# j-wilson/GPflowPILCO

Hardware: AMD Instinct MI355X
Metric: moment_matched_rollout_step_elements_per_sec (higher is better)
Workload: dtype f32; 1 GPU; C3 (BASELINE configs[2]): N=2000 d=8 D=8 H=40 fp32 drift moment-match step / closed rollout; recipe=baseline: BASELINE.md recipe: lengthscales log-U[0.3,3], GP-prior targets, fresh mu~U[0,1]^d / Sigm~; N=2000, d=8, D=8, H=40, B_per_gpu=256, B_total=256, B_this_rank=256, parallelism=dp1 over B (weak), recipe=baseline, steps_requested=418, diag_pairs=f64, offdiag_pairs=f32

## Files before the change

gpflowpilco_amd/csrc/mm_common.h:

```cpp
#pragma once
#include <stddef.h>
#include <stdint.h>
#include "../../include/gpflowpilco_mm.h"

static inline size_t mm_align_up(size_t x, size_t a) { return (x + a - 1) / a * a; }
static inline int mm_round_up_int(int x, int a) { return (x + a - 1) / a * a; }
static inline size_t mm_elem_size(int dtype) { return dtype == MM_F64 ? 8 : 4; }

#define MM_ISTAGE_NO_ROUTE (1 << 20)
#define MM_ISTAGE_ROUTE (1 << 21)
#define MM_ISTAGE_NO_M56 (1 << 22)
#define MM_ISTAGE_OLD_OFFDIAG (1 << 23)
#define MM_ISTAGE_OLD_SPOLY56 (1 << 24)

#define MM_PW_KERNELS 3

static inline int mm_num_pairs(int L, int flags) {
  return (flags & MM_FULL_OUTPUT_COV) ? L * (L + 1) / 2 : L;
}

static inline int mm_moment_deg(int d) { return d <= 8 ? 4 : 2; }
static inline long long mm_binom(int n, int k) {
  if (k < 0 || k > n) return 0;
  long long r = 1;
  for (int i = 1; i <= k; ++i) r = r * (n - k + i) / i;
  return r;
}
static inline int mm_mono_count(int n, int d) { return (int)mm_binom(d + n - 1, n); }
static inline int mm_mono_offset(int n, int d) { int o = 0; for (int m = 0; m < n; ++m) o += mm_mono_count(m, d); return o; }
static inline size_t mm_rank_table_entries(int d) {
  const int dk = d <= 8 ? 8 : 32, deg = mm_moment_deg(d);
  size_t n = 0, p = 1;
  for (int k = 1; k <= deg; ++k) { p *= dk; n += p; }
  return n;
}
static inline int mm_moment_cols(int d) { return mm_round_up_int(mm_mono_offset(mm_moment_deg(d) + 1, d), 16); }
static inline int mm_moment56_off5(int d) { return d <= 8 ? mm_round_up_int(mm_mono_count(4, d), 128) : 0; }
static inline int mm_moment56_off6(int d) { return d <= 8 ? mm_moment56_off5(d) + mm_round_up_int(mm_mono_count(5, d), 128) : 0; }
static inline int mm_moment56_cols(int d) { return d <= 8 ? mm_moment56_off6(d) + mm_round_up_int(mm_mono_count(6, d), 128) : 0; }
struct MMTab56 { int ins[6], last[6], n_i16, mult2, mult3, n_f32; size_t bytes; };
static inline MMTab56 mm_tab56(int d) {
  MMTab56 t;
  int o = 0;
  for (int m = 0; m < 6; ++m) { t.ins[m] = o; o += mm_mono_count(m, d) * 8; }
  for (int k = 0; k < 6; ++k) { t.last[k] = o; o += mm_mono_count(k, d); }
  t.n_i16 = mm_round_up_int(o, 8);
// ... 225 lines not shown
```

gpflowpilco_amd/csrc/mm_kernels.hip:

```cpp
#include <hip/hip_runtime.h>
#include <math.h>
#include "mm_common.h"
#include "mm_cost.h"
#include "mm_dev.h"
#include "mm_mono.h"

#include <mutex>
#include <unordered_map>
#include "mm_fork.h"

#define MM_ABI_VERSION 2

namespace {
struct MMForkKey {
  int dev; hipStream_t stream;
  bool operator==(const MMForkKey& o) const { return dev == o.dev && stream == o.stream; }
};
struct MMForkKeyHash {
  size_t operator()(const MMForkKey& k) const { return std::hash<const void*>()((const void*)k.stream) * 31u + (size_t)k.dev; }
};
std::mutex g_fork_mu;
std::unordered_map<MMForkKey, MMFork*, MMForkKeyHash> g_forks;

MMFork* mm_fork_lookup(hipStream_t stream, bool create) {
// ... 1108 lines not shown
    if (traj_Sigma) traj_Sigma[(size_t)b * d * d + idx] = (T)v;
  }
  if (lane < d) {
    const double v = (double)mu[(size_t)b * d + lane] + dt * (double)f1[(size_t)b * d + lane];
    mu_out[(size_t)b * d + lane] = (T)v;
    if (traj_mu) traj_mu[(size_t)b * d + lane] = (T)v;
  }
}

template <typename T>
__global__ __launch_bounds__(64) void k_expected_cost(int d, const T* __restrict__ mean, const T* __restrict__ cov,
                                                      const T* __restrict__ target, const T* __restrict__ precis,
                                                      T* __restrict__ cost) {
  extern __shared__ double smem[];
  mm_expected_cost_body<T>(d, mean, cov, target, precis, cost, (int)blockIdx.x, (int)threadIdx.x, smem);
}

extern "C" int mm_mfma_supported(int d);
int mm_mfma_num_slots(int Mp);
int mm_f64_num_slots(int Mp, int diag);
int mm_launch_qred_f64_both(const double* Zc, int Kz, const double* Cm, const double* beta, int M, int L, int Mp, int d, int P, int NS,
                            int Po, int B, int force_worst, const double* qhR, const double* qhC, const double* rowD,
                            const double* colD, const double* w64, const double* q64, const double* rowO, const double* colO,
                            double* partB, double* partC, hipStream_t stream, bool* launched);
int mm_launch_qred_f64(const double* Zc, int Kz, const double* Cm, const double* beta, int M, int L, int Mp, int d,
                       int P, int NS, int p0, int npairs, int B, int diag, int lowp, int force_worst,
                       const double* w, const double* q, const double* rowA, const double* colB,
                       double* partB, double* partC, hipStream_t stream);
int mm_launch_qred_mfma(const char* packed, const MMModelLayout& ml, char* ws, const MMWorkspaceLayout& wl,
                        int B, int L, int d, int flags, hipStream_t stream);
int mm_launch_route(const char* packed, const MMModelLayout& ml, char* ws, const MMWorkspaceLayout& wl, int B, int L, int M,
                    int d, int flags, int agg, double* out, int32_t* status, hipStream_t stream);
int mm_launch_moments(const char* packed, const MMModelLayout& ml, char* ws, const MMWorkspaceLayout& wl,
                      int B, int L, int d, const void* mu_f32, int flags, hipStream_t stream);

int mm_launch_pack56(char* packed, const MMModelLayout& lay, int L, int M, int d, const double* Z, hipStream_t s);

#define MM_CHECK_LAUNCH() do { hipError_t e_ = hipGetLastError(); if (e_ != hipSuccess) return (int)e_; } while (0)

static int mm_check_common(const void* packed, int L, int M, int d, int dtype, int B) {
  if (!packed) return MM_E_ARG;
  if (L <= 0 || M <= 0 || d <= 0 || B <= 0) return MM_E_ARG;
  if (d > MM_DMAX) return MM_E_DIM;
  if (dtype != MM_F32 && dtype != MM_F64) return MM_E_DTYPE;
  return 0;
}

static inline int mm_dk(int d) { return d <= 4 ? 4 : d <= 8 ? 8 : d <= 16 ? 16 : 32; }

extern "C" int mm_abi_version(void) { return MM_ABI_VERSION; }

extern "C" size_t mm_packed_model_bytes(int L, int M, int d, int dtype, int with_C) {
  if (L <= 0 || M <= 0 || d <= 0 || d > MM_DMAX) return 0;
  return mm_model_layout(L, M, d, dtype, with_C).total;
}

extern "C" size_t mm_workspace_bytes(int B, int L, int M, int d, int dtype, int flags) {
  if (B <= 0 || L <= 0 || M <= 0 || d <= 0 || d > MM_DMAX) return 0;
  return mm_workspace_layout(B, L, M, d, dtype, flags).total;
}

template <typename T>
static int mm_pack_model_t(char* packed, const MMModelLayout& lay, int L, int M, int d,
                           const double* Z, const double* ls, const double* var, const double* beta,
                           const double* C, const double* mean_c, hipStream_t s) {
  const int sorted = M > MM_SORT_MIN_M ? 1 : 0;
  if (sorted) {
// ... 78 lines not shown
      if (ns > nblk) ns = nblk;
      return ns < 1 ? 1 : ns;
    };
#define MM_PAIRVEC_ARGS                                                                                                     \
    (const double*)(packed + ml.Zt64), (const double*)(packed + ml.zbar), ls2, L, M, wl.Mp, d, wl.P, mu, pairmat,            \
    (const double*)(ws + wl.rho1), (double*)(ws + wl.rowD), (double*)(ws + wl.colD), (T*)(ws + wl.rowO), (T*)(ws + wl.colO), \
    (const double*)(ws + wl.w64), (double*)(ws + wl.whR), (double*)(ws + wl.whC), amax,                                      \
    (const double*)(ws + wl.q64), (double*)(ws + wl.qhR), (double*)(ws + wl.qhC), (flags & MM_MODEL_UNCERTAINTY) ? 1 : 0, nblk, \
    (const double*)(ws + wl.lq), (const double*)(packed + ml.beta64), (const double*)(packed + ml.zmax2),                       \
    ((sizeof(T) == 4 && d <= 8) ? (unsigned short*)(ws + wl.wsp) : (unsigned short*)nullptr),                                \
    (unsigned char*)(ws + wl.gflag), (float*)(ws + wl.gmax2), ((flags & (MM_FORCE_WORST_TIER | MM_ISTAGE_NO_M56)) ? 0 : 1)
    auto pairvec = [&](int p0, int npairs, hipStream_t st) {
      if (npairs <= 0) return;
      if constexpr (DK <= 8) {
        hipLaunchKernelGGL((k_pairvec_reg<T, DK>), dim3(nsplit_for(npairs), npairs, B), dim3(256), 0, st, MM_PAIRVEC_ARGS, p0);
      } else {
        hipLaunchKernelGGL((k_pairvec<T, DK>), dim3(nsplit_for(npairs), npairs, B), dim3(256), 0, st, MM_PAIRVEC_ARGS, p0);
      }
    };
    pairvec(0, L, s);
    MM_CHECK_LAUNCH();
    if (wl.Po > 0) {
      MMFork* fork = (joins && (long long)wl.P * B >= 512) ? mm_fork_get(s) : nullptr;
      hipStream_t s2 = s;
      if (fork) {
        hipError_t ef = hipEventRecord(fork->fork, s);
        if (ef == hipSuccess) ef = hipStreamWaitEvent(fork->s2, fork->fork, 0);
        if (ef != hipSuccess) return (int)ef;
        s2 = fork->s2;
      }
      pairvec(L, wl.Po, s2);
      int rcs = 0;
      { hipError_t e_ = hipGetLastError(); if (e_ != hipSuccess) rcs = (int)e_; }
      if (!rcs && sizeof(T) == 4) rcs = mm_launch_moments(packed, ml, ws, wl, B, L, d, (const void*)mu, flags, s2);
      if (fork) {
        hipError_t ej = hipEventRecord(fork->join, fork->s2);
        if (rcs) { if (ej == hipSuccess) (void)hipStreamWaitEvent(s, fork->join, 0); return rcs; }
        if (ej != hipSuccess) return (int)ej;
      }
      if (rcs) return rcs;
    }
#undef MM_PAIRVEC_ARGS
  }
  MM_CHECK_LAUNCH();
  return 0;
}

template <typename T, int DK>
static int mm_Q_reduce_t(const char* packed, const MMModelLayout& ml, bool has_C, char* ws, const MMWorkspaceLayout& wl,
                         int L, int M, int d, int B, int flags, double jitter, T* Sff, int32_t* status, hipStream_t s) {
  const int with_unc = (flags & MM_MODEL_UNCERTAINTY) ? 1 : 0;
  const int full = (flags & MM_FULL_OUTPUT_COV) ? 1 : 0;
  if (with_unc && !has_C) return MM_E_NO_C;
  const double* Cm = with_unc ? (const double*)(packed + ml.Cm) : nullptr;
  double* partB = (double*)(ws + wl.partB);
  double* partC = (double*)(ws + wl.partC);
  const int nrb = (wl.Mp + MM_GEN_ROWS - 1) / MM_GEN_ROWS, ncb = (wl.Mp + MM_GEN_COLS - 1) / MM_GEN_COLS;
  const bool generic = (flags & MM_FORCE_GENERIC) != 0;
  const bool use_mfma32 = sizeof(T) == 4 && !generic && mm_mfma_supported(d);
  const int ns_gen = nrb * ncb;
  const int nsB_diag = generic ? ns_gen : mm_f64_num_slots(wl.Mp, 1), nsC = nsB_diag;
  const int nsB_off = generic ? ns_gen : (sizeof(T) == 4 ? (use_mfma32 ? mm_mfma_num_slots(wl.Mp) : ns_gen)
                                                         : mm_f64_num_slots(wl.Mp, 0));
  int stages = flags & (MM_STAGE_DIAG | MM_STAGE_OFFDIAG | MM_STAGE_FINALIZE);
  if (!stages) stages = MM_STAGE_DIAG | MM_STAGE_OFFDIAG | MM_STAGE_FINALIZE;
  const bool routes = use_mfma32 && wl.Po > 0 && !(flags & (MM_FORCE_WORST_TIER | MM_NO_ROUTE));
  bool both = false;
// ... 224 lines not shown
```

gpflowpilco_amd/csrc/mm_moments.hip:

```cpp
#include <hip/hip_runtime.h>
#include <math.h>
#include "mm_common.h"
#include "mm_mono.h"

typedef double f64x4m __attribute__((ext_vector_type(4)));

#define MM_GEMM_RB 64
#define MM_GEMM_NB 128
#define MM_GEMM_KB 32
#define MM_GEMM_AS 34
#define MM_GEMM_BS 144

__device__ __forceinline__ void mm_decode_pair_m(int p, int L, int& a, int& a2) {
  int r = p - L, i = 0;
  while (r >= L - 1 - i) { r -= L - 1 - i; ++i; }
  a = i; a2 = i + 1 + r;
}

__global__ __launch_bounds__(256) __attribute__((amdgpu_waves_per_eu(2, 2))) void k_wmom_gemm(const double* __restrict__ whR, const double* __restrict__ whC,
                                                      const double* __restrict__ Zm, int KMp, int L, int Mp, int B, int Po,
                                                      int nrb, int ncb, int nwork, int col_deg3,
                                                      const unsigned int* __restrict__ amaxc, const double* __restrict__ zmax2,
                                                      const int* __restrict__ gperm, double* __restrict__ mom) {
  const int orig = blockIdx.x;
  const int xcd = orig & 7, slot = orig >> 3;
  const int qn = nwork >> 3, rn = nwork & 7;
  int wi = (xcd < rn ? xcd * (qn + 1) : rn * (qn + 1) + (xcd - rn) * qn) + slot;
  const int rb = wi % nrb; wi /= nrb;
  const int ks = wi % MM_MOM_SPLIT; wi /= MM_MOM_SPLIT;
  const int cb = wi % ncb; wi /= ncb;
  const int a = wi;
  const int R = (L - 1) * B;
  auto row_item = [&](int r, int& b, int& po, int& side, int& acol) {
    const int which = r / B;
    b = r - which * B;
    const int ap = which < a ? which : which + 1;
    const int lo = ap < a ? ap : a, hi = ap < a ? a : ap;
    po = lo * (L - 1) - lo * (lo - 1) / 2 + (hi - lo - 1);
    side = ap < a ? 1 : 0;
    acol = hi;
  };
  const double* tab = Zm + (size_t)a * Mp * KMp;
  const int tid = threadIdx.x, wv = tid >> 6, lane = tid & 63, l15 = lane & 15, kq = lane >> 4;
  const int* perm = nullptr;
  if (cb * MM_GEMM_NB >= col_deg3) {
    if (gperm != nullptr) {
      if (rb * MM_GEMM_RB >= gperm[(size_t)L * R + a]) return;
      perm = gperm + (size_t)a * R;
    } else {
      const int r = rb * MM_GEMM_RB + lane;
      bool c = false;
      if (amaxc != nullptr && r < R) {
        int b, po, side, acol;
        row_item(r, b, po, side, acol);
        c = mm_item_collapsed(amaxc[(size_t)b * Po + po]);
      }
      if (!__any(c)) return;
    }
  }
  const int kslice = Mp / MM_MOM_SPLIT;
  const int k_begin = ks * kslice, nkb = kslice / MM_GEMM_KB;

  __shared__ double As[MM_GEMM_RB * MM_GEMM_AS];
  __shared__ double Bs[MM_GEMM_KB * MM_GEMM_BS];

  const int ar = tid >> 2, ak = (tid & 3) * 8;
  int arow = rb * MM_GEMM_RB + ar;
  arow = arow < R ? arow : R - 1;
  int ab, apo, aside, aacol;
  row_item(perm ? perm[arow] : arow, ab, apo, aside, aacol);
  const double* aptr = (aside ? whC : whR) + ((size_t)ab * Po + apo) * Mp + k_begin + ak;

  const int bk = tid >> 3, bc = (tid & 7) * 16;
  const int col0 = cb * MM_GEMM_NB + bc;
  const bool bvalid = col0 < KMp;
  const double* bptr = tab + (size_t)(k_begin + bk) * KMp + (bvalid ? col0 : 0);
  double2 ra[4], rbv[8];
  auto load_regs = [&](int kb) {
    const double* ap = aptr + kb * MM_GEMM_KB;
#pragma unroll
    for (int i = 0; i < 4; ++i) ra[i] = *reinterpret_cast<const double2*>(ap + 2 * i);
    const double* bp = bptr + (size_t)kb * MM_GEMM_KB * KMp;
#pragma unroll
    for (int i = 0; i < 8; ++i) rbv[i] = *reinterpret_cast<const double2*>(bp + 2 * i);
  };
  f64x4m acc[4][2];
#pragma unroll
  for (int rt = 0; rt < 4; ++rt)
#pragma unroll
    for (int ct = 0; ct < 2; ++ct) acc[rt][ct] = (f64x4m){0.0, 0.0, 0.0, 0.0};

  load_regs(0);
  for (int kb = 0; kb < nkb; ++kb) {
    __syncthreads();
#pragma unroll
    for (int i = 0; i < 4; ++i) *reinterpret_cast<double2*>(&As[ar * MM_GEMM_AS + ak + 2 * i]) = ra[i];
#pragma unroll
    for (int i = 0; i < 8; ++i)
      *reinterpret_cast<double2*>(&Bs[bk * MM_GEMM_BS + bc + 2 * ((i + (tid & 7)) & 7)]) = bvalid ? rbv[i] : make_double2(0.0, 0.0);
    __syncthreads();
    load_regs(kb + 1 < nkb ? kb + 1 : kb);
#pragma unroll
    for (int s = 0; s < MM_GEMM_KB / 4; ++s) {
      double av[4], bv[2];
#pragma unroll
      for (int rt = 0; rt < 4; ++rt) av[rt] = As[(rt * 16 + l15) * MM_GEMM_AS + 4 * s + kq];
#pragma unroll
      for (int ct = 0; ct < 2; ++ct)
        bv[ct] = Bs[(4 * s + kq) * MM_GEMM_BS + wv * 32 + ct * 16 + 2 * (((l15 >> 1) + 2 * wv + ct) & 7) + (l15 & 1)];
#pragma unroll
      for (int rt = 0; rt < 4; ++rt)
#pragma unroll
        for (int ct = 0; ct < 2; ++ct)
          acc[rt][ct] = __builtin_amdgcn_mfma_f64_16x16x4f64(av[rt], bv[ct], acc[rt][ct], 0, 0, 0);
    }
  }
#pragma unroll
  for (int rt = 0; rt < 4; ++rt)
#pragma unroll
    for (int r = 0; r < 4; ++r) {
      const int row = rb * MM_GEMM_RB + rt * 16 + kq + 4 * r;
      if (row >= R) continue;
      int b, po, side, acol;
      row_item(perm ? perm[row] : row, b, po, side, acol);
      double* o = mom + ((((size_t)b * Po + po) * 2 + side) * MM_MOM_SPLIT + ks) * KMp;
#pragma unroll
      for (int ct = 0; ct < 2; ++ct) {
        const int col = cb * MM_GEMM_NB + wv * 32 + ct * 16 + l15;
        if (col < KMp) o[col] = acc[rt][ct][r];
      }
    }
}

__global__ __launch_bounds__(1024) void k_wmom_perm(const unsigned int* __restrict__ amaxc, const double* __restrict__ zmax2, int L, int B,
                                                    int Po, int* __restrict__ gperm) {
  const int a = blockIdx.x, tid = threadIdx.x, wv = tid >> 6, lane = tid & 63;
  const int R = (L - 1) * B;
  __shared__ int wsum[3][16];
  __shared__ int tot[3];
  int* out = gperm + (size_t)a * R;
  int cnt[3] = {0, 0, 0};
  auto cls_of = [&](int r) {
    const int which = r / B, b = r - which * B;
    const int ap = which < a ? which : which + 1;
    const int lo = ap < a ? ap : a, hi = ap < a ? a : ap;
    const int po = lo * (L - 1) - lo * (lo - 1) / 2 + (hi - lo - 1);
    const unsigned int ac = amaxc[(size_t)b * Po + po];
    const float x2 = mm_collapse_bound2(ac, zmax2[hi]);
    return !mm_item_collapsed(ac) ? 3 : (x2 > MM_C6_X5_2 ? 0 : (x2 > MM_C6_X4_2 ? 1 : 2));
  };
  for (int r = tid; r < R; r += 1024) { const int c = cls_of(r); if (c < 3) ++cnt[c]; }
#pragma unroll
  for (int c = 0; c < 3; ++c) {
#pragma unroll
    for (int off = 32; off > 0; off >>= 1) cnt[c] += __shfl_down(cnt[c], off, 64);
    if (lane == 0) wsum[c][wv] = cnt[c];
  }
  __syncthreads();
  if (tid < 3) { int t = 0; for (int w = 0; w < 16; ++w) t += wsum[tid][w]; tot[tid] = t; }
  __syncthreads();
  int ofs[3] = {0, tot[0], tot[0] + tot[1]};
  int ofs_n = 0;
// ... 19 lines not shown
      before[k] += wb; ctot[k] = ct;
      nfront_before += before[k]; nfront_tot += ct;
    }
    if (in) {
      if (c < 3) out[ofs[c] + before[c]] = r;
      else out[R - 1 - (ofs_n + (tid - nfront_before))] = r;
    }
    const int nin = R - r0 < 1024 ? R - r0 : 1024;
#pragma unroll
    for (int k = 0; k < 3; ++k) ofs[k] += ctot[k];
    ofs_n += nin - nfront_tot;
  }
  if (tid == 0) {
    gperm[(size_t)L * R + a] = tot[0] + tot[1] + tot[2];
    gperm[(size_t)L * R + L + a] = tot[0] + tot[1];
    gperm[(size_t)L * R + 2 * L + a] = tot[0];
  }
}

__device__ __forceinline__ double mm_block_sum256m(double v, double* red) {
#pragma unroll
  for (int off = 32; off > 0; off >>= 1) v += __shfl_down(v, off, 64);
  __syncthreads();
  if ((threadIdx.x & 63) == 0) red[threadIdx.x >> 6] = v;
  __syncthreads();
  return red[0] + red[1] + red[2] + red[3];
}

template <int DK, int LB>
__global__ __launch_bounds__(256) void k_spoly(const double* __restrict__ mom, int KMp, const double* __restrict__ pairmat,
                                               const double* __restrict__ zbar, const double* __restrict__ zmax2,
                                               const unsigned int* __restrict__ amax, const unsigned int* __restrict__ amaxc,
                                               const float* __restrict__ mu,
                                               int L, int d, int P, int deg, int allow_collapse,
                                               int off1, int off2, int off3, int off4, const short* __restrict__ rtab,
                                               double c0, double c1, double* __restrict__ s12) {
  extern __shared__ double sm[];
  const int po = blockIdx.x, b = blockIdx.y, tid = threadIdx.x;
  const int Po = P - L, p = L + po;
  int a, a2;
  mm_decode_pair_m(p, L, a, a2);
  const int dn = 1 << (LB * deg);
#define MM_PADI(i_) ((i_) + ((i_) >> 5))
  double* T = sm;
  double* U = T + MM_PADI(dn);
  double* nh = U + MM_PADI(dn >> LB);
  double* qh = nh + KMp;
  double* Gs = qh + KMp;
  double* dmu = Gs + DK * DK;
  __shared__ double red[4];
  {
    const double* nm = mom + (((size_t)b * Po + po) * 2 + 0) * MM_MOM_SPLIT * KMp;
    const double* qm = mom + (((size_t)b * Po + po) * 2 + 1) * MM_MOM_SPLIT * KMp;
    for (int k = tid; k < KMp; k += 256) {
      double sn = 0.0, sq = 0.0;
#pragma unroll
      for (int t = 0; t < MM_MOM_SPLIT; ++t) { sn += nm[t * KMp + k]; sq += qm[t * KMp + k]; }
      nh[k] = sn; qh[k] = sq;
    }
    const double* pm = pairmat + ((size_t)b * P + p) * (d * d + 1);
    for (int idx = tid; idx < DK * DK; idx += 256) {
      const int i = idx >> LB, j = idx & (DK - 1);
      Gs[idx] = (i < d && j < d) ? pm[i * d + j] : 0.0;
    }
    const bool rcen = mm_rows_recentred(amax[(size_t)b * Po + po]);
    if (tid < DK) dmu[tid] = (tid < d && !rcen) ? (double)mu[(size_t)b * d + tid] - zbar[a * d + tid] : 0.0;
  }
  __syncthreads();
  const bool coll = allow_collapse && deg >= 3 && mm_item_collapsed(amaxc[(size_t)b * Po + po]);
  const int nmax = coll ? deg : 2;
  double Gr[DK == 8 ? 64 : 1];
  if constexpr (DK == 8) {
#pragma unroll
    for (int i = 0; i < 64; ++i) Gr[i] = Gs[i];
  }
  double total = 0.0;
  for (int n = nmax; n >= 1; --n) {
    const double an = n == 1 ? 1.0 : n == 2 ? 0.5 : n == 3 ? c0 : c1;
    const int dsz = 1 << (LB * n);
    const int offn = n == 1 ? off1 : n == 2 ? off2 : n == 3 ? off3 : off4;
    const short* rtn = rtab + (((1 << (LB * n)) - DK) / (DK - 1));
    for (int idx = tid; idx < dsz; idx += 256) {
      const int r = rtn[idx];
      T[MM_PADI(idx)] = r >= 0 ? qh[offn + r] : 0.0;
    }
    __syncthreads();
    for (int t = 0; t < n; ++t) {
      const int sh = LB * t, nfib = dsz >> LB;
      for (int f = tid; f < nfib; f += 256) {
        const int lo = f & ((1 << sh) - 1), hi = f >> sh;
        const int base = (hi << (sh + LB)) + lo;
        double v[DK];
#pragma unroll
        for (int l = 0; l < DK; ++l) v[l] = T[MM_PADI(base + (l << sh))];
        if constexpr (DK == 8) {
#pragma unroll
          for (int k = 0; k < 8; ++k) {
            double s = 0.0;
#pragma unroll
            for (int l = 0; l < 8; ++l) s = fma(Gr[k * 8 + l], v[l], s);
            T[MM_PADI(base + (k << sh))] = s;
          }
        } else {
// ... 18 lines not shown
      const short* rtk = rtab + (k ? (((1 << (LB * k)) - DK) / (DK - 1)) : 0);
      for (int idx = tid; idx < ksz; idx += 256) {
        const int r = k ? rtk[idx] : 0;
        if (r >= 0) part = fma(cur[MM_PADI(idx)], nh[offk + r], part);
      }
      total = fma(an * sign_binom, part, total);
      if (k == 0) break;
      const int nsz = ksz >> LB;
      for (int idx = tid; idx < nsz; idx += 256) {
        double s = 0.0;
#pragma unroll
        for (int l = 0; l < DK; ++l) s = fma(cur[MM_PADI(l * nsz + idx)], dmu[l], s);
        oth[MM_PADI(idx)] = s;
      }
      __syncthreads();
      double* tsw = cur; cur = oth; oth = tsw;
      ksz = nsz;
      sign_binom = -sign_binom * (double)k / (double)(n - k + 1);
    }
    __syncthreads();
  }
  const double tot = mm_block_sum256m(total, red);
  if (tid == 0) s12[(size_t)b * Po + po] = tot + nh[0] * qh[0];
#undef MM_PADI
}

int mm_launch_wmom_full(const char* packed, const MMModelLayout& ml, char* ws, const MMWorkspaceLayout& wl,
                        int B, int L, int d, hipStream_t stream) {
  const int nrb = ((L - 1) * B + MM_GEMM_RB - 1) / MM_GEMM_RB, ncb = (ml.KMp + MM_GEMM_NB - 1) / MM_GEMM_NB;
  const long long nwork_ll = (long long)L * ncb * MM_MOM_SPLIT * nrb;
  if (nwork_ll <= 0 || nwork_ll > 0x7fffffffLL) return MM_E_DIM;
  hipLaunchKernelGGL(k_wmom_gemm, dim3((int)nwork_ll), dim3(256), 0, stream, (const double*)(ws + wl.whR),
                     (const double*)(ws + wl.whC), (const double*)(packed + ml.Zm), ml.KMp, L, wl.Mp, B, wl.Po, nrb, ncb,
                     (int)nwork_ll, 0x7fffffff , (const unsigned int*)nullptr, (const double*)(packed + ml.zmax2),
                     (const int*)nullptr, (double*)(ws + wl.mom));
  hipError_t e = hipGetLastError();
  return e == hipSuccess ? 0 : (int)e;
}

int mm_launch_moments56(const char* packed, const MMModelLayout& ml, char* ws, const MMWorkspaceLayout& wl,
                        int B, int L, int d, int allow, int old_spoly56, hipStream_t stream);

int mm_launch_moments(const char* packed, const MMModelLayout& ml, char* ws, const MMWorkspaceLayout& wl,
                      int B, int L, int d, const void* mu_f32, int flags, hipStream_t stream) {
  const double* Zm = (const double*)(packed + ml.Zm);
  double* mom = (double*)(ws + wl.mom);
  const int deg = mm_moment_deg(d) >= 4 ? 3 : mm_moment_deg(d);
  const int ncol_fwd = mm_mono_offset(deg + 1, d);
  const int nrb = ((L - 1) * B + MM_GEMM_RB - 1) / MM_GEMM_RB, ncb = (ncol_fwd + MM_GEMM_NB - 1) / MM_GEMM_NB;
  const long long nwork_ll = (long long)L * ncb * MM_MOM_SPLIT * nrb;
  if (nwork_ll <= 0 || nwork_ll > 0x7fffffffLL) return MM_E_DIM;
  const int nwork = (int)nwork_ll;
  const int allow = (flags & (MM_FORCE_WORST_TIER | MM_ISTAGE_NO_M56)) ? 0 : 1;
  const int col_deg3 = mm_mono_offset(3, d);
  const bool some = allow && mm_moment_deg(d) >= 4;
  if (some) {
    hipLaunchKernelGGL(k_wmom_perm, dim3(L), dim3(1024), 0, stream, (const unsigned int*)(ws + wl.amaxc),
                       (const double*)(packed + ml.zmax2), L, B, wl.Po, (int*)(ws + wl.gperm));
    hipError_t ep = hipGetLastError();
    if (ep != hipSuccess) return (int)ep;
  }
  hipLaunchKernelGGL(k_wmom_gemm, dim3(nwork), dim3(256), 0, stream, (const double*)(ws + wl.whR),
                     (const double*)(ws + wl.whC), Zm, ml.KMp, L, wl.Mp, B, wl.Po, nrb, ncb, nwork, col_deg3,
                     some ? (const unsigned int*)(ws + wl.amaxc) : (const unsigned int*)nullptr,
                     (const double*)(packed + ml.zmax2), some ? (const int*)(ws + wl.gperm) : (const int*)nullptr, mom);
  hipError_t e = hipGetLastError();
  if (e != hipSuccess) return (int)e;
  const int off1 = mm_mono_offset(1, d), off2 = mm_mono_offset(2, d), off3 = mm_mono_offset(3, d), off4 = mm_mono_offset(4, d);
#define MM_SPOLY(DK_, LB_)                                                                                                       \
  do {                                                                                                                          \
    const int dn_ = 1 << (LB_ * deg);                                                                                           \
    const int up_ = dn_ >> LB_;                                                                                                 \
    const size_t shm_ = (size_t)(dn_ + (dn_ >> 5) + up_ + (up_ >> 5) + 2 * ml.KMp + DK_ * DK_ + DK_ + 8) * sizeof(double);      \
    hipLaunchKernelGGL((k_spoly<DK_, LB_>), dim3(wl.Po, B), dim3(256), shm_, stream, (const double*)mom, ml.KMp,                \
                       (const double*)(ws + wl.pairmat), (const double*)(packed + ml.zbar), (const double*)(packed + ml.zmax2), \
                       (const unsigned int*)(ws + wl.amax), (const unsigned int*)(ws + wl.amaxc), (const float*)mu_f32, L, d, wl.P, deg, allow, off1, off2, off3, off4, \
                       (const short*)(packed + ml.rtab),                                                                        \
                       (double)MM_C6_C0, (double)MM_C6_C1, (double*)(ws + wl.s12));                                             \
  } while (0)
  if (d <= 8) MM_SPOLY(8, 3); else MM_SPOLY(32, 5);
#undef MM_SPOLY
  e = hipGetLastError();
  if (e != hipSuccess) return (int)e;
  if (flags & MM_ISTAGE_NO_M56) {
    if (mm_moment56_cols(d) <= 0 || wl.Po <= 0) return 0;
    const hipError_t em = hipMemsetAsync(ws + wl.s56, 0xFF, (size_t)B * wl.Po * sizeof(double), stream);
    if (em != hipSuccess) return (int)em;
    const hipError_t es = hipMemsetAsync(ws + wl.estS, 0, (size_t)B * wl.Po * sizeof(float), stream);
    return es == hipSuccess ? 0 : (int)es;
  }
  return mm_launch_moments56(packed, ml, ws, wl, B, L, d, some ? 1 : 0, (flags & MM_ISTAGE_OLD_SPOLY56) ? 1 : 0, stream);
}

__global__ void k_offdiag_stats(const unsigned int* __restrict__ amax, const double* __restrict__ zmax2,
                                const unsigned char* __restrict__ gflag, int ng, int L, int Po, int n,
                                int32_t* __restrict__ out) {
  const int idx = blockIdx.x * blockDim.x + threadIdx.x;
  bool c = false, in = false, part = false;
  int groups = 0;
  if (idx < n) {
    int a, a2;
    mm_decode_pair_m(L + idx % Po, L, a, a2);
    const float b2 = mm_collapse_bound2(amax[idx], zmax2[a2]);
    c = b2 <= MM_COLLAPSE_BOUND2;
    in = b2 <= MM_INSIDE_BOUND2;
    part = !c && mm_item_collapsed(amax[n + idx]);
    for (int g = 0; g < ng; ++g) groups += gflag[(size_t)idx * ng + g] ? 1 : 0;
  }
  const unsigned long long m = __ballot(c), mi = __ballot(in), mp = __ballot(part);
  if ((threadIdx.x & 63) == 0 && m) atomicAdd(out, (int)__popcll(m));
  if ((threadIdx.x & 63) == 0 && mi) atomicAdd(out + 2, (int)__popcll(mi));
  if ((threadIdx.x & 63) == 0 && mp) atomicAdd(out + 4, (int)__popcll(mp));
#pragma unroll
  for (int off = 32; off > 0; off >>= 1) groups += __shfl_down(groups, off, 64);
  if ((threadIdx.x & 63) == 0 && groups) atomicAdd(out + 5, groups);
  if (idx == 0) out[1] = n;
}

extern "C" int mm_offdiag_stats(const void* packed, size_t packed_bytes, int L, int M, int d, int dtype, int B, int flags,
                                const void* workspace, size_t workspace_bytes, int32_t* out, void* stream) {
  if (!packed || !workspace || !out || L <= 0 || M <= 0 || d <= 0 || d > MM_DMAX || B <= 0) return MM_E_ARG;
  const MMModelLayout ml = mm_model_layout(L, M, d, dtype, 1);
  const MMWorkspaceLayout wl = mm_workspace_layout(B, L, M, d, dtype, flags);
  if (packed_bytes < ml.Cm || workspace_bytes < wl.total) return MM_E_WORKSPACE;
// ... 16 lines not shown
```

gpflowpilco_amd/csrc/mm_moments6.hip:

```cpp
#include <hip/hip_runtime.h>
#include <math.h>
#include "mm_common.h"
#include "mm_mono.h"
#include "mm_f32_tile.h"
#include <atomic>
#include <type_traits>

__device__ __forceinline__ void mm6_decode_pair_o(int lp, int L, int& a, int& a2) {
  int r = lp, i = 0;
  while (r >= L - 1 - i) { r -= L - 1 - i; ++i; }
  a = i; a2 = i + 1 + r;
}

__global__ __launch_bounds__(256) void k_pack_zm56(char* packed, MMModelLayout lay, int L, int M, int d, int N56p,
                                                   const double* __restrict__ Z) {
  const int c = blockIdx.x, a = blockIdx.y, tid = threadIdx.x;
  const int n4 = mm_binom_i(d + 3, 4), n5 = mm_binom_i(d + 4, 5), n6 = mm_binom_i(d + 5, 6);
  const int off5 = ((n4 + 127) / 128) * 128;
  const int off6 = off5 + ((n5 + 127) / 128) * 128;
  const double* zbar = (const double*)(packed + lay.zbar) + (size_t)a * d;
  unsigned short* oh = (unsigned short*)(packed + lay.Zm56) + (((size_t)a * 2 + 0) * N56p + c) * lay.Mp;
  unsigned short* om = (unsigned short*)(packed + lay.Zm56) + (((size_t)a * 2 + 1) * N56p + c) * lay.Mp;
  int n = 0, k[6] = {0, 0, 0, 0, 0, 0};
  if (c < n4) { n = 4; mm_mono_unrank(c, 4, k); }
// ... 43 lines not shown
  for (int n = 2; n <= 3; ++n) {
    const int ns = mm_binom_i(d + n - 1, n);
    for (int I = tid; I < ns; I += 256) {
      int k[6] = {0, 0, 0, 0, 0, 0};
      mm_mono_unrank(I, n, k);
      double mult = 1.0;
      int run = 0;
      for (int u = 0; u < n; ++u) {
        mult *= (double)(u + 1);
        run = (u > 0 && k[u] == k[u - 1]) ? run + 1 : 1;
        mult /= (double)run;
      }
      f32[(n == 2 ? t.mult2 : t.mult3) + I] = (float)mult;
    }
  }
}

int mm_launch_pack56(char* packed, const MMModelLayout& lay, int L, int M, int d, const double* Z, hipStream_t s) {
  const int N56p = mm_moment56_cols(d);
  if (N56p <= 0) return 0;
  hipLaunchKernelGGL(k_pack_zm56, dim3(N56p, L), dim3(256), 0, s, packed, lay, L, M, d, N56p, Z);
  hipError_t e = hipGetLastError();
  if (e != hipSuccess) return (int)e;
  hipLaunchKernelGGL(k_pack_tab56, dim3(1), dim3(256), 0, s, packed, lay, d, mm_tab56(d));
  e = hipGetLastError();
  return e == hipSuccess ? 0 : (int)e;
}

#define MM6_TB 128
#define MM6_KB 32
#define MM6_STAGE_BYTES 32768

__global__ __launch_bounds__(256, 2) void k_wmom56_gemm(const unsigned short* __restrict__ wsp, const unsigned short* __restrict__ Zm56,
                                                        int N56p, int L, int Mp, int B, int Po, int nrb, int ncb, int nwork, int cb5, int cb6,
                                                        const int* __restrict__ gperm, float* __restrict__ mom56) {
  const int orig = blockIdx.x;
  const int xcd = orig & 7, slot = orig >> 3;
  const int qn = nwork >> 3, rn = nwork & 7;
  int wi = (xcd < rn ? xcd * (qn + 1) : rn * (qn + 1) + (xcd - rn) * qn) + slot;
  const int rb = wi % nrb; wi /= nrb;
  const int cb = wi % ncb; wi /= ncb;
  const int a = wi;
  const int R = (L - 1) * B;
  const int ncoll = gperm[(size_t)L * R + (cb < cb5 ? 0 : (cb < cb6 ? 1 : 2)) * L + a];
  if (rb * MM6_TB >= ncoll) return;
  const int* perm = gperm + (size_t)a * R;
  extern __shared__ __align__(1024) char lds[];
  int* orow = reinterpret_cast<int*>(lds + 2 * MM6_STAGE_BYTES);
  const int tid = threadIdx.x, wv = tid >> 6, lane = tid & 63, l31 = lane & 31, h = lane >> 5;
  auto row_item = [&](int r) {
    const int which = r / B, b = r - which * B;
    const int ap = which < a ? which : which + 1;
    const int lo = ap < a ? ap : a, hi = ap < a ? a : ap;
    const int po = lo * (L - 1) - lo * (lo - 1) / 2 + (hi - lo - 1);
    return ((b * Po + po) << 1) | (ap < a ? 1 : 0);
  };
  if (tid < MM6_TB) {
    const int r = rb * MM6_TB + tid;
    orow[tid] = r < ncoll ? row_item(perm[r]) : -1;
  }
  const bool isB = wv >= 2;
  const int part = wv & 1;
  unsigned int src_off[8];
#pragma unroll
  for (int i = 0; i < 8; ++i) {
    const int row = i * 16 + (lane >> 2);
    const int lc = (lane & 3) ^ ((row >> 2) & 3);
    if (isB) {
      src_off[i] = (unsigned int)((((size_t)a * 2 + part) * N56p + (size_t)cb * MM6_TB + row) * Mp) + lc * 8;
    } else {
      int r = rb * MM6_TB + row;
      r = r < ncoll ? r : ncoll - 1;
      src_off[i] = (unsigned int)(((size_t)row_item(perm[r]) * 2 + part) * Mp) + lc * 8;
    }
  }
  const unsigned short* src = isB ? Zm56 : wsp;
  auto stage = [&](int kb, int buf) {
    char* dst = lds + buf * MM6_STAGE_BYTES + (isB ? 16384 : 0) + part * 8192;
#pragma unroll
    for (int i = 0; i < 8; ++i)
      __builtin_amdgcn_global_load_lds((const __attribute__((address_space(1))) void*)(src + src_off[i] + kb * MM6_KB),
                                       (__attribute__((address_space(3))) void*)(dst + i * 1024), 16, 0, 0);
  };
  const int wr = wv >> 1, wc = wv & 1;
  f32x16 acc[2][2];
#pragma unroll
  for (int rt = 0; rt < 2; ++rt)
#pragma unroll
    for (int ct = 0; ct < 2; ++ct)
#pragma unroll
      for (int e = 0; e < 16; ++e) acc[rt][ct][e] = 0.0f;
  int fragA[2], fragB[2];
#pragma unroll
  for (int t = 0; t < 2; ++t) {
    fragA[t] = (wr * 64 + t * 32 + l31) * 64;
    fragB[t] = 16384 + (wc * 64 + t * 32 + l31) * 64;
  }
  const int swz = (l31 >> 2) & 3;
  const int nkb = Mp / MM6_KB;
  stage(0, 0);
  for (int kb = 0; kb < nkb; ++kb) {
    __syncthreads();
    if (kb + 1 < nkb) stage(kb + 1, (kb + 1) & 1);
    const char* base = lds + (kb & 1) * MM6_STAGE_BYTES;
#pragma unroll
    for (int ks = 0; ks < 2; ++ks) {
      const int ch = ((ks * 2 + h) ^ swz) * 16;
      bf16x8 Ah[2], Am[2], Th[2], Tm[2];
#pragma unroll
      for (int t = 0; t < 2; ++t) {
        Ah[t] = *reinterpret_cast<const bf16x8*>(base + fragA[t] + ch);
        Am[t] = *reinterpret_cast<const bf16x8*>(base + 8192 + fragA[t] + ch);
        Th[t] = *reinterpret_cast<const bf16x8*>(base + fragB[t] + ch);
        Tm[t] = *reinterpret_cast<const bf16x8*>(base + 8192 + fragB[t] + ch);
      }
#pragma unroll
      for (int rt = 0; rt < 2; ++rt)
#pragma unroll
        for (int ct = 0; ct < 2; ++ct) {
          acc[rt][ct] = __builtin_amdgcn_mfma_f32_32x32x16_bf16(Am[rt], Th[ct], acc[rt][ct], 0, 0, 0);
          acc[rt][ct] = __builtin_amdgcn_mfma_f32_32x32x16_bf16(Ah[rt], Tm[ct], acc[rt][ct], 0, 0, 0);
          acc[rt][ct] = __builtin_amdgcn_mfma_f32_32x32x16_bf16(Ah[rt], Th[ct], acc[rt][ct], 0, 0, 0);
        }
    }
  }
#pragma unroll
  for (int rt = 0; rt < 2; ++rt)
#pragma unroll
    for (int e = 0; e < 16; ++e) {
      const int item = orow[wr * 64 + rt * 32 + 8 * (e >> 2) + 4 * h + (e & 3)];
      if (item < 0) continue;
      float* o = mom56 + (size_t)item * N56p + (size_t)cb * MM6_TB + wc * 64 + l31;
// ... 488 lines not shown
        G[4 * q] = g4.x; G[4 * q + 1] = g4.y; G[4 * q + 2] = g4.z; G[4 * q + 3] = g4.w;
      }
    };
    float acc4 = 0.0f, dummy = 0.0f;
    const float* Q4 = nq + sy[4];
    const float* N4 = nq;
    load_G(1);
    mm6_do<D8, 0, false, 0, NC0, NW, 4, 0>(Q4, Bf4, sy, tabi, tb, d, G, nullptr, 0, dummy, wave, lane);
    __syncthreads();
    mm6_do<D8, 1, false, 1, 1, NW, 3, 37>(Bf4, X4, sy, tabi, tb, d, G, mult2, xs4, dummy, wave, lane);
    __syncthreads();
    load_G(0);
    mm6_do<D8, 0, true, 0, NC0, NW, 4, 0>(N4, Bf4, sy, tabi, tb, d, G, nullptr, 0, dummy, wave, lane);
    __syncthreads();
    mm6_do<D8, 1, true, 2, 1, NW, 3, 37>(Bf4, X4, sy, tabi, tb, d, G, nullptr, xs4, acc4, wave, lane);
    double tot = (double)MM_C6_C1 * (double)acc4;
#pragma unroll
    for (int off = 32; off > 0; off >>= 1) {
      tot += __shfl_down(tot, off, 64); s2r += __shfl_down(s2r, off, 64); s2c += __shfl_down(s2c, off, 64);
    }
    if (lane == 0) { redd[wave * 3 + 0] = tot; redd[wave * 3 + 1] = s2r; redd[wave * 3 + 2] = s2c; }
    __syncthreads();
    if (tid == 0) {
      double t = 0.0, r2 = 0.0, c2 = 0.0;
      for (int w = 0; w < NW; ++w) { t += redd[w * 3]; r2 += redd[w * 3 + 1]; c2 += redd[w * 3 + 2]; }
      s56[item] = t;
      estS[item] = mm6_estS(bound2, false, false, r2, c2);
    }
    __syncthreads();
  }
}

int mm_launch_moments56(const char* packed, const MMModelLayout& ml, char* ws, const MMWorkspaceLayout& wl,
                        int B, int L, int d, int allow, int old_spoly56, hipStream_t stream) {
  const int N56p = mm_moment56_cols(d);
  if (N56p <= 0 || wl.Po <= 0) return 0;
  if (allow) {
    const int nrb = ((L - 1) * B + MM6_TB - 1) / MM6_TB, ncb = N56p / MM6_TB;
    const long long nwork_ll = (long long)L * ncb * nrb;
    if (nwork_ll <= 0 || nwork_ll > 0x7fffffffLL) return MM_E_DIM;
    if ((size_t)B * wl.Po * 4 * wl.Mp >= 0xffffffffull || (size_t)L * 2 * N56p * wl.Mp >= 0xffffffffull) return MM_E_DIM;
    const size_t shm = 2 * MM6_STAGE_BYTES + MM6_TB * sizeof(int);
    static std::atomic<unsigned long long> attr_done{0ull};
    int dev = 0;
    if (hipGetDevice(&dev) != hipSuccess) dev = 64;
    const unsigned long long bit = (dev >= 0 && dev < 64) ? (1ull << dev) : 0ull;
    if (!bit || !(attr_done.load() & bit)) {
      const hipError_t ea = hipFuncSetAttribute((const void*)k_wmom56_gemm, hipFuncAttributeMaxDynamicSharedMemorySize, (int)shm);
      if (ea != hipSuccess) return (int)ea;
      attr_done.fetch_or(bit);
    }
    hipLaunchKernelGGL(k_wmom56_gemm, dim3((int)nwork_ll), dim3(256), shm, stream, (const unsigned short*)(ws + wl.wsp),
                       (const unsigned short*)(packed + ml.Zm56), N56p, L, wl.Mp, B, wl.Po, nrb, ncb, (int)nwork_ll,
                       mm_moment56_off5(d) / MM6_TB, mm_moment56_off6(d) / MM6_TB,
                       (const int*)(ws + wl.gperm), (float*)(ws + wl.mom56));
    hipError_t e = hipGetLastError();
    if (e != hipSuccess) return (int)e;
  }
  const int nitem = B * wl.Po;
  int* ilist = (int*)(ws + wl.ilist);
  {
    const hipError_t em = hipMemsetAsync(ilist, 0, 16, stream);
    if (em != hipSuccess) return (int)em;
  }
  hipLaunchKernelGGL(k_item_classes, dim3((nitem + 255) / 256), dim3(256), 0, stream, (const unsigned int*)(ws + wl.amaxc),
                     (const double*)(packed + ml.zmax2), L, wl.Po, nitem, allow, ilist, (double*)(ws + wl.s56), (float*)(ws + wl.estS));
  {
    const hipError_t ec = hipGetLastError();
    if (ec != hipSuccess) return (int)ec;
  }
  if (!allow) return 0;
  int sy[7];
  for (int k = 0; k < 7; ++k) sy[k] = mm_mono_count(k, d);
  size_t nfl = (size_t)2 * (sy[4] + sy[5] + sy[6]) + (size_t)sy[3] * (sy[3] + 1) + (size_t)sy[2] * sy[4] + (size_t)sy[1] * sy[5] + 6 * MM6_WAVES + 128 + 16
               + (size_t)sy[1] * sy[3] + (size_t)sy[2] * (sy[2] + 1);
  nfl = (nfl + 1) & ~(size_t)1;
  const size_t shm = nfl * sizeof(float);
  static std::atomic<unsigned long long> attr2_done{0ull};
  static std::atomic<int> ncu_cached[64];
  int dev = 0;
  if (hipGetDevice(&dev) != hipSuccess) dev = 64;
  const unsigned long long bit2 = (dev >= 0 && dev < 64) ? (1ull << dev) : 0ull;
  int ncu = bit2 ? ncu_cached[dev].load() : 0;
  if (!bit2 || !(attr2_done.load() & bit2)) {
    hipError_t ea = hipFuncSetAttribute((const void*)k_spoly56<false>, hipFuncAttributeMaxDynamicSharedMemorySize, 160 * 1024);
    if (ea == hipSuccess) ea = hipFuncSetAttribute((const void*)k_spoly56<true>, hipFuncAttributeMaxDynamicSharedMemorySize, 160 * 1024);
// ... 27 lines not shown
```

Before: 42100 rollout step-elements/s (B*H per rollout second).

## Trim moment GEMMs to live K rows and live monomial columns

The f64 moment GEMM and the bf16 56-moment GEMM now stop their K loop at the real inducing-point count M instead of the padded Mp. The f64 GEMM also limits its columns to the live monomial count, using a light single-row-tile MFMA path when few column tiles remain. The spoly reduction reads only up to the needed monomial offset. This removes wasted MFMA work and memory traffic on padding, at the cost of more branching and per-wave divergence in tile counts. An escape flag keeps the old extents available.

```diff
diff --git a/gpflowpilco_amd/csrc/mm_common.h b/gpflowpilco_amd/csrc/mm_common.h
--- a/gpflowpilco_amd/csrc/mm_common.h
+++ b/gpflowpilco_amd/csrc/mm_common.h
@@ -12,6 +12,7 @@
 #define MM_ISTAGE_NO_M56 (1 << 22)
 #define MM_ISTAGE_OLD_OFFDIAG (1 << 23)
 #define MM_ISTAGE_OLD_SPOLY56 (1 << 24)
+#define MM_ISTAGE_OLD_EXTENT (1 << 25)
 
 #define MM_PW_KERNELS 3
 
diff --git a/gpflowpilco_amd/csrc/mm_kernels.hip b/gpflowpilco_amd/csrc/mm_kernels.hip
--- a/gpflowpilco_amd/csrc/mm_kernels.hip
+++ b/gpflowpilco_amd/csrc/mm_kernels.hip
@@ -1164,7 +1164,7 @@
 int mm_launch_route(const char* packed, const MMModelLayout& ml, char* ws, const MMWorkspaceLayout& wl, int B, int L, int M,
                     int d, int flags, int agg, double* out, int32_t* status, hipStream_t stream);
 int mm_launch_moments(const char* packed, const MMModelLayout& ml, char* ws, const MMWorkspaceLayout& wl,
-                      int B, int L, int d, const void* mu_f32, int flags, hipStream_t stream);
+                      int B, int L, int M, int d, const void* mu_f32, int flags, hipStream_t stream);
 
 int mm_launch_pack56(char* packed, const MMModelLayout& lay, int L, int M, int d, const double* Z, hipStream_t s);
 
@@ -1309,7 +1309,7 @@
       pairvec(L, wl.Po, s2);
       int rcs = 0;
       { hipError_t e_ = hipGetLastError(); if (e_ != hipSuccess) rcs = (int)e_; }
-      if (!rcs && sizeof(T) == 4) rcs = mm_launch_moments(packed, ml, ws, wl, B, L, d, (const void*)mu, flags, s2);
+      if (!rcs && sizeof(T) == 4) rcs = mm_launch_moments(packed, ml, ws, wl, B, L, M, d, (const void*)mu, flags, s2);
       if (fork) {
         hipError_t ej = hipEventRecord(fork->join, fork->s2);
         if (rcs) { if (ej == hipSuccess) (void)hipStreamWaitEvent(s, fork->join, 0); return rcs; }
diff --git a/gpflowpilco_amd/csrc/mm_moments.hip b/gpflowpilco_amd/csrc/mm_moments.hip
--- a/gpflowpilco_amd/csrc/mm_moments.hip
+++ b/gpflowpilco_amd/csrc/mm_moments.hip
@@ -2,6 +2,7 @@
 #include <math.h>
 #include "mm_common.h"
 #include "mm_mono.h"
+#include <type_traits>
 
 typedef double f64x4m __attribute__((ext_vector_type(4)));
 
@@ -19,7 +20,7 @@
 
 __global__ __launch_bounds__(256) __attribute__((amdgpu_waves_per_eu(2, 2))) void k_wmom_gemm(const double* __restrict__ whR, const double* __restrict__ whC,
                                                       const double* __restrict__ Zm, int KMp, int L, int Mp, int B, int Po,
-                                                      int nrb, int ncb, int nwork, int col_deg3,
+                                                      int nrb, int ncb, int nwork, int col_deg3, int ncol_live, int klive,
                                                       const unsigned int* __restrict__ amaxc, const double* __restrict__ zmax2,
                                                       const int* __restrict__ gperm, double* __restrict__ mom) {
   const int orig = blockIdx.x;
@@ -41,7 +42,8 @@
     acol = hi;
   };
   const double* tab = Zm + (size_t)a * Mp * KMp;
-  const int tid = threadIdx.x, wv = tid >> 6, lane = tid & 63, l15 = lane & 15, kq = lane >> 4;
+  const int tid = threadIdx.x, lane = tid & 63, l15 = lane & 15, kq = lane >> 4;
+  const int wv = __builtin_amdgcn_readfirstlane(tid >> 6);
   const int* perm = nullptr;
   if (cb * MM_GEMM_NB >= col_deg3) {
     if (gperm != nullptr) {
@@ -59,7 +61,15 @@
     }
   }
   const int kslice = Mp / MM_MOM_SPLIT;
-  const int k_begin = ks * kslice, nkb = kslice / MM_GEMM_KB;
+  const int k_begin = ks * kslice;
+  int nkb = (klive - k_begin + MM_GEMM_KB - 1) / MM_GEMM_KB;
+  nkb = nkb < 0 ? 0 : (nkb < kslice / MM_GEMM_KB ? nkb : kslice / MM_GEMM_KB);
+  const int ncl = ncol_live < KMp ? ncol_live : KMp;
+  int nlt = (ncl - cb * MM_GEMM_NB) / 16;
+  nlt = nlt > 8 ? 8 : nlt;
+  const bool light = nlt <= 4;
+  int nct = nlt - 2 * wv;
+  nct = nct < 0 ? 0 : (nct > 2 ? 2 : nct);
 
   __shared__ double As[MM_GEMM_RB * MM_GEMM_AS];
   __shared__ double Bs[MM_GEMM_KB * MM_GEMM_BS];
@@ -73,16 +83,20 @@
 
   const int bk = tid >> 3, bc = (tid & 7) * 16;
   const int col0 = cb * MM_GEMM_NB + bc;
-  const bool bvalid = col0 < KMp;
+  const bool bvalid = col0 < ncl;
   const double* bptr = tab + (size_t)(k_begin + bk) * KMp + (bvalid ? col0 : 0);
   double2 ra[4], rbv[8];
+#pragma unroll
+  for (int i = 0; i < 8; ++i) rbv[i] = make_double2(0.0, 0.0);
   auto load_regs = [&](int kb) {
     const double* ap = aptr + kb * MM_GEMM_KB;
 #pragma unroll
     for (int i = 0; i < 4; ++i) ra[i] = *reinterpret_cast<const double2*>(ap + 2 * i);
     const double* bp = bptr + (size_t)kb * MM_GEMM_KB * KMp;
-#pragma unroll
-    for (int i = 0; i < 8; ++i) rbv[i] = *reinterpret_cast<const double2*>(bp + 2 * i);
+    if (bvalid) {
+#pragma unroll
+      for (int i = 0; i < 8; ++i) rbv[i] = *reinterpret_cast<const double2*>(bp + 2 * i);
+    }
   };
   f64x4m acc[4][2];
 #pragma unroll
@@ -90,30 +104,74 @@
 #pragma unroll
     for (int ct = 0; ct < 2; ++ct) acc[rt][ct] = (f64x4m){0.0, 0.0, 0.0, 0.0};
 
+#define MM_GEMM_BCOL(c_) ((c_) * 16 + 2 * (((l15 >> 1) + (c_)) & 7) + (l15 & 1))
+  auto mma = [&](auto nct_tag) {
+    constexpr int NCT = decltype(nct_tag)::value;
+#pragma unroll
+    for (int s = 0; s < MM_GEMM_KB / 4; ++s) {
+      double av[4], bv[NCT];
+#pragma unroll
+      for (int rt = 0; rt < 4; ++rt) av[rt] = As[(rt * 16 + l15) * MM_GEMM_AS + 4 * s + kq];
+#pragma unroll
+      for (int ct = 0; ct < NCT; ++ct) bv[ct] = Bs[(4 * s + kq) * MM_GEMM_BS + MM_GEMM_BCOL(2 * wv + ct)];
+#pragma unroll
+      for (int rt = 0; rt < 4; ++rt)
+#pragma unroll
+        for (int ct = 0; ct < NCT; ++ct)
+          acc[rt][ct] = __builtin_amdgcn_mfma_f64_16x16x4f64(av[rt], bv[ct], acc[rt][ct], 0, 0, 0);
+    }
+  };
+  auto mma_light = [&](auto nlt_tag) {
+    constexpr int NLT = decltype(nlt_tag)::value;
+#pragma unroll
+    for (int s = 0; s < MM_GEMM_KB / 4; ++s) {
+      const double av = As[(wv * 16 + l15) * MM_GEMM_AS + 4 * s + kq];
+      double bv[NLT];
+#pragma unroll
+      for (int j = 0; j < NLT; ++j) bv[j] = Bs[(4 * s + kq) * MM_GEMM_BS + MM_GEMM_BCOL(j)];
+#pragma unroll
+      for (int j = 0; j < NLT; ++j) acc[j][0] = __builtin_amdgcn_mfma_f64_16x16x4f64(av, bv[j], acc[j][0], 0, 0, 0);
+    }
+  };
   load_regs(0);
   for (int kb = 0; kb < nkb; ++kb) {
     __syncthreads();
 #pragma unroll
     for (int i = 0; i < 4; ++i) *reinterpret_cast<double2*>(&As[ar * MM_GEMM_AS + ak + 2 * i]) = ra[i];
-#pragma unroll
-    for (int i = 0; i < 8; ++i)
-      *reinterpret_cast<double2*>(&Bs[bk * MM_GEMM_BS + bc + 2 * ((i + (tid & 7)) & 7)]) = bvalid ? rbv[i] : make_double2(0.0, 0.0);
+    if (bvalid) {
+#pragma unroll
+      for (int i = 0; i < 8; ++i)
+        *reinterpret_cast<double2*>(&Bs[bk * MM_GEMM_BS + bc + 2 * ((i + (tid & 7)) & 7)]) = rbv[i];
+    }
     __syncthreads();
     load_regs(kb + 1 < nkb ? kb + 1 : kb);
-#pragma unroll
-    for (int s = 0; s < MM_GEMM_KB / 4; ++s) {
-      double av[4], bv[2];
-#pragma unroll
-      for (int rt = 0; rt < 4; ++rt) av[rt] = As[(rt * 16 + l15) * MM_GEMM_AS + 4 * s + kq];
-#pragma unroll
-      for (int ct = 0; ct < 2; ++ct)
-        bv[ct] = Bs[(4 * s + kq) * MM_GEMM_BS + wv * 32 + ct * 16 + 2 * (((l15 >> 1) + 2 * wv + ct) & 7) + (l15 & 1)];
-#pragma unroll
-      for (int rt = 0; rt < 4; ++rt)
-#pragma unroll
-        for (int ct = 0; ct < 2; ++ct)
-          acc[rt][ct] = __builtin_amdgcn_mfma_f64_16x16x4f64(av[rt], bv[ct], acc[rt][ct], 0, 0, 0);
-    }
+    if (light) {
+      switch (nlt) {
+        case 1: mma_light(std::integral_constant<int, 1>{}); break;
+        case 2: mma_light(std::integral_constant<int, 2>{}); break;
+        case 3: mma_light(std::integral_constant<int, 3>{}); break;
+        default: mma_light(std::integral_constant<int, 4>{}); break;
+      }
+    } else if (nct == 2) {
+      mma(std::integral_constant<int, 2>{});
+    } else if (nct == 1) {
+      mma(std::integral_constant<int, 1>{});
+    }
+  }
+#undef MM_GEMM_BCOL
+  if (light) {
+#pragma unroll
+    for (int r = 0; r < 4; ++r) {
+      const int row = rb * MM_GEMM_RB + wv * 16 + kq + 4 * r;
+      if (row >= R) continue;
+      int b, po, side, acol;
+      row_item(perm ? perm[row] : row, b, po, side, acol);
+      double* o = mom + ((((size_t)b * Po + po) * 2 + side) * MM_MOM_SPLIT + ks) * KMp + cb * MM_GEMM_NB + l15;
+#pragma unroll
+      for (int j = 0; j < 4; ++j)
+        if (j < nlt) o[j * 16] = acc[j][0][r];
+    }
+    return;
   }
 #pragma unroll
   for (int rt = 0; rt < 4; ++rt)
@@ -127,7 +185,7 @@
 #pragma unroll
       for (int ct = 0; ct < 2; ++ct) {
         const int col = cb * MM_GEMM_NB + wv * 32 + ct * 16 + l15;
-        if (col < KMp) o[col] = acc[rt][ct][r];
+        if (ct < nct) o[col] = acc[rt][ct][r];
       }
     }
 }
@@ -213,7 +271,7 @@
                                                const double* __restrict__ zbar, const double* __restrict__ zmax2,
                                                const unsigned int* __restrict__ amax, const unsigned int* __restrict__ amaxc,
                                                const float* __restrict__ mu,
-                                               int L, int d, int P, int deg, int allow_collapse,
+                                               int L, int d, int P, int deg, int allow_collapse, int old_extent,
                                                int off1, int off2, int off3, int off4, const short* __restrict__ rtab,
                                                double c0, double c1, double* __restrict__ s12) {
   extern __shared__ double sm[];
@@ -230,10 +288,13 @@
   double* Gs = qh + KMp;
   double* dmu = Gs + DK * DK;
   __shared__ double red[4];
+  const bool coll = allow_collapse && deg >= 3 && mm_item_collapsed(amaxc[(size_t)b * Po + po]);
+  const int nmax = coll ? deg : 2;
+  const int kload = old_extent ? KMp : (nmax >= 3 ? off4 : off3);
   {
     const double* nm = mom + (((size_t)b * Po + po) * 2 + 0) * MM_MOM_SPLIT * KMp;
     const double* qm = mom + (((size_t)b * Po + po) * 2 + 1) * MM_MOM_SPLIT * KMp;
-    for (int k = tid; k < KMp; k += 256) {
+    for (int k = tid; k < kload; k += 256) {
       double sn = 0.0, sq = 0.0;
 #pragma unroll
       for (int t = 0; t < MM_MOM_SPLIT; ++t) { sn += nm[t * KMp + k]; sq += qm[t * KMp + k]; }
@@ -248,8 +309,6 @@
     if (tid < DK) dmu[tid] = (tid < d && !rcen) ? (double)mu[(size_t)b * d + tid] - zbar[a * d + tid] : 0.0;
   }
   __syncthreads();
-  const bool coll = allow_collapse && deg >= 3 && mm_item_collapsed(amaxc[(size_t)b * Po + po]);
-  const int nmax = coll ? deg : 2;
   double Gr[DK == 8 ? 64 : 1];
   if constexpr (DK == 8) {
 #pragma unroll
@@ -334,17 +393,17 @@
   if (nwork_ll <= 0 || nwork_ll > 0x7fffffffLL) return MM_E_DIM;
   hipLaunchKernelGGL(k_wmom_gemm, dim3((int)nwork_ll), dim3(256), 0, stream, (const double*)(ws + wl.whR),
                      (const double*)(ws + wl.whC), (const double*)(packed + ml.Zm), ml.KMp, L, wl.Mp, B, wl.Po, nrb, ncb,
-                     (int)nwork_ll, 0x7fffffff , (const unsigned int*)nullptr, (const double*)(packed + ml.zmax2),
+                     (int)nwork_ll, 0x7fffffff , ml.KMp, wl.Mp, (const unsigned int*)nullptr, (const double*)(packed + ml.zmax2),
                      (const int*)nullptr, (double*)(ws + wl.mom));
   hipError_t e = hipGetLastError();
   return e == hipSuccess ? 0 : (int)e;
 }
 
 int mm_launch_moments56(const char* packed, const MMModelLayout& ml, char* ws, const MMWorkspaceLayout& wl,
-                        int B, int L, int d, int allow, int old_spoly56, hipStream_t stream);
+                        int B, int L, int d, int allow, int old_spoly56, int klive, hipStream_t stream);
 
 int mm_launch_moments(const char* packed, const MMModelLayout& ml, char* ws, const MMWorkspaceLayout& wl,
-                      int B, int L, int d, const void* mu_f32, int flags, hipStream_t stream) {
+                      int B, int L, int M, int d, const void* mu_f32, int flags, hipStream_t stream) {
   const double* Zm = (const double*)(packed + ml.Zm);
   double* mom = (double*)(ws + wl.mom);
   const int deg = mm_moment_deg(d) >= 4 ? 3 : mm_moment_deg(d);
@@ -353,6 +412,9 @@
   const long long nwork_ll = (long long)L * ncb * MM_MOM_SPLIT * nrb;
   if (nwork_ll <= 0 || nwork_ll > 0x7fffffffLL) return MM_E_DIM;
   const int nwork = (int)nwork_ll;
+  const bool old_extent = (flags & MM_ISTAGE_OLD_EXTENT) != 0;
+  const int ncol_live = old_extent ? ncb * MM_GEMM_NB : mm_round_up_int(ncol_fwd, 16);
+  const int klive = old_extent ? wl.Mp : M;
   const int allow = (flags & (MM_FORCE_WORST_TIER | MM_ISTAGE_NO_M56)) ? 0 : 1;
   const int col_deg3 = mm_mono_offset(3, d);
   const bool some = allow && mm_moment_deg(d) >= 4;
@@ -363,7 +425,7 @@
     if (ep != hipSuccess) return (int)ep;
   }
   hipLaunchKernelGGL(k_wmom_gemm, dim3(nwork), dim3(256), 0, stream, (const double*)(ws + wl.whR),
-                     (const double*)(ws + wl.whC), Zm, ml.KMp, L, wl.Mp, B, wl.Po, nrb, ncb, nwork, col_deg3,
+                     (const double*)(ws + wl.whC), Zm, ml.KMp, L, wl.Mp, B, wl.Po, nrb, ncb, nwork, col_deg3, ncol_live, klive,
                      some ? (const unsigned int*)(ws + wl.amaxc) : (const unsigned int*)nullptr,
                      (const double*)(packed + ml.zmax2), some ? (const int*)(ws + wl.gperm) : (const int*)nullptr, mom);
   hipError_t e = hipGetLastError();
@@ -376,7 +438,7 @@
     const size_t shm_ = (size_t)(dn_ + (dn_ >> 5) + up_ + (up_ >> 5) + 2 * ml.KMp + DK_ * DK_ + DK_ + 8) * sizeof(double);      \
     hipLaunchKernelGGL((k_spoly<DK_, LB_>), dim3(wl.Po, B), dim3(256), shm_, stream, (const double*)mom, ml.KMp,                \
                        (const double*)(ws + wl.pairmat), (const double*)(packed + ml.zbar), (const double*)(packed + ml.zmax2), \
-                       (const unsigned int*)(ws + wl.amax), (const unsigned int*)(ws + wl.amaxc), (const float*)mu_f32, L, d, wl.P, deg, allow, off1, off2, off3, off4, \
+                       (const unsigned int*)(ws + wl.amax), (const unsigned int*)(ws + wl.amaxc), (const float*)mu_f32, L, d, wl.P, deg, allow, old_extent ? 1 : 0, off1, off2, off3, off4, \
                        (const short*)(packed + ml.rtab),                                                                        \
                        (double)MM_C6_C0, (double)MM_C6_C1, (double*)(ws + wl.s12));                                             \
   } while (0)
@@ -391,7 +453,7 @@
     const hipError_t es = hipMemsetAsync(ws + wl.estS, 0, (size_t)B * wl.Po * sizeof(float), stream);
     return es == hipSuccess ? 0 : (int)es;
   }
-  return mm_launch_moments56(packed, ml, ws, wl, B, L, d, some ? 1 : 0, (flags & MM_ISTAGE_OLD_SPOLY56) ? 1 : 0, stream);
+  return mm_launch_moments56(packed, ml, ws, wl, B, L, d, some ? 1 : 0, (flags & MM_ISTAGE_OLD_SPOLY56) ? 1 : 0, klive, stream);
 }
 
 __global__ void k_offdiag_stats(const unsigned int* __restrict__ amax, const double* __restrict__ zmax2,
diff --git a/gpflowpilco_amd/csrc/mm_moments6.hip b/gpflowpilco_amd/csrc/mm_moments6.hip
--- a/gpflowpilco_amd/csrc/mm_moments6.hip
+++ b/gpflowpilco_amd/csrc/mm_moments6.hip
@@ -99,7 +99,7 @@
 #define MM6_STAGE_BYTES 32768
 
 __global__ __launch_bounds__(256, 2) void k_wmom56_gemm(const unsigned short* __restrict__ wsp, const unsigned short* __restrict__ Zm56,
-                                                        int N56p, int L, int Mp, int B, int Po, int nrb, int ncb, int nwork, int cb5, int cb6,
+                                                        int N56p, int L, int Mp, int klive, int B, int Po, int nrb, int ncb, int nwork, int cb5, int cb6,
                                                         const int* __restrict__ gperm, float* __restrict__ mom56) {
   const int orig = blockIdx.x;
   const int xcd = orig & 7, slot = orig >> 3;
@@ -164,7 +164,7 @@
     fragB[t] = 16384 + (wc * 64 + t * 32 + l31) * 64;
   }
   const int swz = (l31 >> 2) & 3;
-  const int nkb = Mp / MM6_KB;
+  const int nkb = (klive + MM6_KB - 1) / MM6_KB;
   stage(0, 0);
   for (int kb = 0; kb < nkb; ++kb) {
     __syncthreads();
@@ -719,7 +719,7 @@
 }
 
 int mm_launch_moments56(const char* packed, const MMModelLayout& ml, char* ws, const MMWorkspaceLayout& wl,
-                        int B, int L, int d, int allow, int old_spoly56, hipStream_t stream) {
+                        int B, int L, int d, int allow, int old_spoly56, int klive, hipStream_t stream) {
   const int N56p = mm_moment56_cols(d);
   if (N56p <= 0 || wl.Po <= 0) return 0;
   if (allow) {
@@ -738,7 +738,7 @@
       attr_done.fetch_or(bit);
     }
     hipLaunchKernelGGL(k_wmom56_gemm, dim3((int)nwork_ll), dim3(256), shm, stream, (const unsigned short*)(ws + wl.wsp),
-                       (const unsigned short*)(packed + ml.Zm56), N56p, L, wl.Mp, B, wl.Po, nrb, ncb, (int)nwork_ll,
+                       (const unsigned short*)(packed + ml.Zm56), N56p, L, wl.Mp, klive, B, wl.Po, nrb, ncb, (int)nwork_ll,
                        mm_moment56_off5(d) / MM6_TB, mm_moment56_off6(d) / MM6_TB,
                        (const int*)(ws + wl.gperm), (float*)(ws + wl.mom56));
     hipError_t e = hipGetLastError();
```

After: 42460 rollout step-elements/s (B*H per rollout second), median of 6. About the same (+0.9%).
